# NVlabs/FoundationPose

Hardware: NVIDIA H100
Metric: pose-hypotheses/sec at 640x480 RGB-D, 252 hyp, 5 refine iters (higher is better)
Workload: dtype f16

## Files before the change

foundationpose_b200/csrc/fp_attn_tc.cu:

```cuda
#include "fp_attn.cuh"
#include "fp_common.cuh"
#include "fp_gemm.cuh"
#include "fp_wgmma.cuh"

namespace fp {

int encode_map_f16(CUtensorMap* map, const void* base, int rank, const uint64_t* dims, const uint64_t* strides_bytes,
                   const uint32_t* box);
int num_sms();

namespace {

constexpr int T = 400;
constexpr int DH = 128;
constexpr int kQTiles = (T + 127) / 128;
constexpr int kKeys = 80;
constexpr int kChunks = T / kKeys;
constexpr int kKVSlab = kKeys * 128;
constexpr int kKVStage = 4 * kKVSlab;
constexpr int kKVStages = 3;
constexpr int kQSlab = 128 * 128;
constexpr int kQStage = 2 * kQSlab;
constexpr int kQStages = 2;
constexpr int kOffKV = 0;
constexpr int kOffQ = kOffKV + kKVStages * kKVStage;
constexpr int kOffBar = kOffQ + kQStages * kQStage;
constexpr int kSmem = kOffBar + 256 + 1024;
constexpr int kThreadsTc = 384;

__device__ __forceinline__ void tma_load_3d(const CUtensorMap* map, uint64_t* bar, void* dst, int c0, int c1, int c2) {
  asm volatile(
      "cp.async.bulk.tensor.3d.shared::cluster.global.mbarrier::complete_tx::bytes [%0], [%1, {%3, %4, %5}], [%2];" ::"r"(
          smem_u32(dst)),
      "l"(reinterpret_cast<uint64_t>(map)), "r"(smem_u32(bar)), "r"(c0), "r"(c1), "r"(c2)
      : "memory");
}
__device__ __forceinline__ void tma_store_4d(const CUtensorMap* map, const void* src, int c0, int c1, int c2, int c3) {
  asm volatile("cp.async.bulk.tensor.4d.global.shared::cta.bulk_group [%0, {%2, %3, %4, %5}], [%1];" ::"l"(
                   reinterpret_cast<uint64_t>(map)),
               "r"(smem_u32(src)), "r"(c0), "r"(c1), "r"(c2), "r"(c3)
               : "memory");
}

struct TcParams {
  int q_col, k_col, v_col;
  int group_col_stride;
  float scale_log2e;
  int B, H, G;
};

__global__ void __launch_bounds__(kThreadsTc, 1)
    attn_tc_kernel(const __grid_constant__ CUtensorMap map_kv,
                   const __grid_constant__ CUtensorMap map_q,
                   const __grid_constant__ CUtensorMap map_o,
                   const TcParams p) {
  extern __shared__ uint8_t smem_raw[];
  uint8_t* smem = reinterpret_cast<uint8_t*>((reinterpret_cast<uintptr_t>(smem_raw) + 1023) & ~uintptr_t(1023));
  uint64_t* bars = reinterpret_cast<uint64_t*>(smem + kOffBar);
  uint64_t* q_full = bars;
  uint64_t* q_empty = bars + kQStages;
  uint64_t* kv_full = bars + 2 * kQStages;
  uint64_t* kv_empty = bars + 2 * kQStages + kKVStages;

  const int total = p.B * p.H * p.G * kQTiles;

  if (threadIdx.x == 0) {
    tma_prefetch_desc(&map_kv);
    tma_prefetch_desc(&map_q);
    tma_prefetch_desc(&map_o);
    for (int i = 0; i < kQStages; ++i) {
      mbar_init(&q_full[i], 1);
      mbar_init(&q_empty[i], 2);
    }
    for (int i = 0; i < kKVStages; ++i) {
      mbar_init(&kv_full[i], 1);
      mbar_init(&kv_empty[i], 256);
    }
    mbar_fence_init();
  }
  __syncthreads();
  pdl_trigger();
  pdl_wait();

  auto unit = [&](int u, int& b, int& h, int& g, int& gcol, int& qt) {
    qt = u % kQTiles;
    const int w = u / kQTiles;
    b = w % p.B;
    h = (w / p.B) % p.H;
    g = w / (p.B * p.H);
    gcol = g * p.group_col_stride + h * DH;
  };

  if (threadIdx.x < 128) {
    if (threadIdx.x == 0) {
      int qs = 0, qph = 0, ks = 0, kph = 0;
      for (int u = blockIdx.x; u < total; u += gridDim.x) {
        int b, h, g, gcol, qt;
        unit(u, b, h, g, gcol, qt);
        mbar_wait(&q_empty[qs], qph ^ 1);
        mbar_expect_tx(&q_full[qs], kQStage);
        for (int s = 0; s < 2; ++s)
          tma_load_3d(&map_q, &q_full[qs], smem + kOffQ + qs * kQStage + s * kQSlab, gcol + p.q_col + s * 64, qt * 128, b);
        if (++qs == kQStages) {
          qs = 0;
          qph ^= 1;
        }
        for (int c = 0; c < kChunks; ++c) {
          mbar_wait(&kv_empty[ks], kph ^ 1);
          mbar_expect_tx(&kv_full[ks], kKVStage);
          uint8_t* st = smem + kOffKV + ks * kKVStage;
          for (int s = 0; s < 2; ++s) {
            tma_load_3d(&map_kv, &kv_full[ks], st + s * kKVSlab, gcol + p.k_col + s * 64, c * kKeys, b);
            tma_load_3d(&map_kv, &kv_full[ks], st + (2 + s) * kKVSlab, gcol + p.v_col + s * 64, c * kKeys, b);
          }
          if (++ks == kKVStages) {
            ks = 0;
            kph ^= 1;
          }
        }
      }
    }
    return;
  }

  const int ct = threadIdx.x - 128;
  const int cw = ct >> 7;
  const int lane = threadIdx.x & 31;
  const int r0 = 64 * cw + 16 * ((ct >> 5) & 3) + (lane >> 2);
  const int cq = 2 * (lane & 3);
  const bool leader = ((ct & 127) == 0);
  const float c = p.scale_log2e;
  float s_acc[kKeys / 2], o[DH / 2];
#pragma unroll
  for (int i = 0; i < kKeys / 2; ++i) s_acc[i] = 0.f;
  int qs = 0, qph = 0, ks = 0, kph = 0;
  for (int u = blockIdx.x; u < total; u += gridDim.x) {
    int b, h, g, gcol, qt;
    unit(u, b, h, g, gcol, qt);
#pragma unroll
    for (int i = 0; i < DH / 2; ++i) o[i] = 0.f;
    float m[2] = {-INFINITY, -INFINITY}, l[2] = {0.f, 0.f};
    mbar_wait(&q_full[qs], qph);
    const uint32_t qbase = smem_u32(smem + kOffQ + qs * kQStage) + (uint32_t)cw * 8192u;
    for (int ch = 0; ch < kChunks; ++ch) {
      mbar_wait(&kv_full[ks], kph);
      const uint32_t kvbase = smem_u32(smem + kOffKV + ks * kKVStage);
      wgmma_fence();
#pragma unroll
      for (int kk = 0; kk < 8; ++kk) {
        const int s = kk >> 2, k = kk & 3;
        Wgmma<kKeys>::ss(s_acc, gmma_desc_sw128(qbase + s * kQSlab) + (uint64_t)(2 * k),
                         gmma_desc_sw128(kvbase + s * kKVSlab) + (uint64_t)(2 * k), kk > 0 ? 1u : 0u);
      }
      wgmma_commit();
      wgmma_wait<0>();
      fence_regs(s_acc);
      float mx[2] = {m[0], m[1]};
#pragma unroll
      for (int j = 0; j < kKeys / 8; ++j) {
        mx[0] = fmaxf(mx[0], fmaxf(s_acc[4 * j], s_acc[4 * j + 1]));
        mx[1] = fmaxf(mx[1], fmaxf(s_acc[4 * j + 2], s_acc[4 * j + 3]));
      }
      float mc[2], alpha[2];
#pragma unroll
      for (int hh = 0; hh < 2; ++hh) {
        mx[hh] = fmaxf(mx[hh], __shfl_xor_sync(0xffffffffu, mx[hh], 1));
        mx[hh] = fmaxf(mx[hh], __shfl_xor_sync(0xffffffffu, mx[hh], 2));
        alpha[hh] = exp2f((m[hh] - mx[hh]) * c);
        m[hh] = mx[hh];
        mc[hh] = mx[hh] * c;
        l[hh] *= alpha[hh];
      }
#pragma unroll
      for (int j = 0; j < DH / 8; ++j) {
        o[4 * j] *= alpha[0];
        o[4 * j + 1] *= alpha[0];
        o[4 * j + 2] *= alpha[1];
        o[4 * j + 3] *= alpha[1];
      }
      uint32_t pa[kKeys / 16][4];
#pragma unroll
      for (int j = 0; j < kKeys / 8; ++j) {
#pragma unroll
        for (int hh = 0; hh < 2; ++hh) {
          const float p0 = exp2f(fmaf(s_acc[4 * j + 2 * hh], c, -mc[hh]));
          const float p1 = exp2f(fmaf(s_acc[4 * j + 2 * hh + 1], c, -mc[hh]));
          l[hh] += p0 + p1;
          pa[j >> 1][(j & 1) * 2 + hh] = pack_half2(p0, p1);
        }
      }
      wgmma_fence();
#pragma unroll
      for (int kk = 0; kk < kKeys / 16; ++kk)
        Wgmma<DH>::rs_mn(o, pa[kk], gmma_desc_mn_sw128(kvbase + 2 * kKVSlab + kk * 16 * 128, kKVSlab), 1u);
      wgmma_commit();
      wgmma_wait<0>();
      fence_regs(o);
      mbar_arrive(&kv_empty[ks]);
      if (++ks == kKVStages) {
        ks = 0;
        kph ^= 1;
      }
    }
    float inv[2];
#pragma unroll
    for (int hh = 0; hh < 2; ++hh) {
      l[hh] += __shfl_xor_sync(0xffffffffu, l[hh], 1);
      l[hh] += __shfl_xor_sync(0xffffffffu, l[hh], 2);
      inv[hh] = 1.f / l[hh];
    }
    uint8_t* qst = smem + kOffQ + qs * kQStage;
#pragma unroll
    for (int j = 0; j < DH / 8; ++j) {
#pragma unroll
      for (int hh = 0; hh < 2; ++hh) {
        const int row = r0 + 8 * hh;
        *reinterpret_cast<uint32_t*>(qst + (j >> 3) * kQSlab + row * 128 + ((((uint32_t)j & 7u) ^ (uint32_t)(row & 7)) << 4) +
                                     cq * 2) = pack_half2(o[4 * j + 2 * hh] * inv[hh], o[4 * j + 2 * hh + 1] * inv[hh]);
      }
    }
    asm volatile("fence.proxy.async.shared::cta;" ::: "memory");
    asm volatile("bar.sync %0, 128;" ::"r"(1 + cw) : "memory");
    if (leader) {
      for (int s = 0; s < 2; ++s)
        tma_store_4d(&map_o, qst + s * kQSlab + cw * 8192, h * DH + s * 64, qt * 128 + 64 * cw, b, g);
      asm volatile("cp.async.bulk.commit_group;" ::: "memory");
      asm volatile("cp.async.bulk.wait_group.read 0;" ::: "memory");
      mbar_arrive(&q_empty[qs]);
    }
    if (++qs == kQStages) {
      qs = 0;
      qph ^= 1;
    }
  }
  if (leader) asm volatile("cp.async.bulk.wait_group 0;" ::: "memory");
}

}

int attn_tc_launch(const AttnParams& p, cudaStream_t stream) {
  FP_REQUIRE(p.T == T && p.n_heads == 4, "wgmma attention is specialised for T=400, 4 heads of 128");
  FP_REQUIRE(p.ld_out == 512, "wgmma attention writes [*, 512] rows");
  static std::atomic<unsigned long long> attr_mask{0};
  if (!device_bit_test(attr_mask)) {
    FP_CUDA_OK(cudaFuncSetAttribute(attn_tc_kernel, cudaFuncAttributeMaxDynamicSharedMemorySize, kSmem));
    device_bit_set(attr_mask);
  }
  if (p.B == 0) return 0;
  CUtensorMap mkv, mq, mo;
  const uint64_t E = 2;
  uint64_t d3[3] = {(uint64_t)p.ld, (uint64_t)T, (uint64_t)p.B};
  uint64_t s3[2] = {(uint64_t)p.ld * E, (uint64_t)p.ld * E * T};
  uint32_t bkv[3] = {64, (uint32_t)kKeys, 1}, bq[3] = {64, 128, 1};
  int rc = encode_map_f16(&mkv, p.qkv, 3, d3, s3, bkv);
  if (rc) return rc;
  rc = encode_map_f16(&mq, p.qkv, 3, d3, s3, bq);
  if (rc) return rc;
  uint64_t d4[4] = {512, (uint64_t)T, (uint64_t)p.B, (uint64_t)p.n_groups};
  uint64_t s4[3] = {512 * E, 512 * E * T, (uint64_t)p.out_group_stride * E};
  if (p.n_groups == 1) s4[2] = 512 * E * T * p.B;
  uint32_t bo[4] = {64, 64, 1, 1};
  rc = encode_map_f16(&mo, p.out, 4, d4, s4, bo);
  if (rc) return rc;
  TcParams tp;
  tp.q_col = p.q_off;
  tp.k_col = p.k_off;
  tp.v_col = p.v_off;
  tp.group_col_stride = p.group_col_stride;
  tp.scale_log2e = p.scale * 1.4426950408889634f;
  tp.B = p.B;
  tp.H = p.n_heads;
  tp.G = p.n_groups;
  const int total = p.B * p.n_heads * p.n_groups * kQTiles;
  const int sms = num_sms();
  FP_REQUIRE(sms > 0, "no CUDA device");
  dim3 grid(total < sms ? total : sms);
  FP_CUDA_OK(launch_pdl(attn_tc_kernel, grid, dim3(kThreadsTc), kSmem, stream, 1, mkv, mq, mo, tp));
  note_launches(1);
  FP_CUDA_OK(cudaGetLastError());
  return 0;
}

}
```

foundationpose_b200/csrc/fp_common.cuh:

```cuda
#pragma once
#include <cuda.h>
#include <cuda_fp16.h>
#include <cuda_runtime.h>
#include <stdint.h>
#include <stdio.h>
#include <string.h>

#include <atomic>

namespace fp {

void note_launches(int n);
unsigned long long launch_count();
void set_capturing(bool on);
inline bool device_bit_test(const std::atomic<unsigned long long>& m) {
  int d = 0;
  cudaGetDevice(&d);
  return (m.load(std::memory_order_acquire) >> (d & 63)) & 1ull;
}
inline void device_bit_set(std::atomic<unsigned long long>& m) {
  int d = 0;
  cudaGetDevice(&d);
  m.fetch_or(1ull << (d & 63), std::memory_order_release);
}
int num_sms();

void set_last_error(const char* fmt, ...);
int check_device_ptr(const void* p, const char* what, const char* fn = "fp_pose_errors");
#define FP_CUDA_OK(expr)                                                                   \
  do {                                                                                     \
    cudaError_t _e = (expr);                                                               \
    if (_e != cudaSuccess) {                                                               \
      fp::set_last_error("%s:%d: %s -> %s", __FILE__, __LINE__, #expr, cudaGetErrorString(_e)); \
      return -2;                                                                           \
    }                                                                                      \
  } while (0)
#define FP_REQUIRE(cond, ...)                                                              \
  do {                                                                                     \
    if (!(cond)) {                                                                         \
      fp::set_last_error(__VA_ARGS__);                                                     \
      return -1;                                                                           \
    }                                                                                      \
  } while (0)
#define FP_TRY(expr)     \
  do {                   \
    int _rc = (expr);    \
    if (_rc) return _rc; \
  } while (0)

bool pdl_enabled();
void pdl_skip_next();

template <typename... KArgs, typename... Args>
inline cudaError_t launch_pdl(void (*kernel)(KArgs...), dim3 grid, dim3 block, size_t smem, cudaStream_t stream,
                              int cluster_x, Args... args) {
  cudaLaunchConfig_t cfg;
  memset(&cfg, 0, sizeof(cfg));
  cfg.gridDim = grid;
  cfg.blockDim = block;
  cfg.dynamicSmemBytes = smem;
  cfg.stream = stream;
  cudaLaunchAttribute attr[2];
  int na = 0;
  if (cluster_x > 1) {
    attr[na].id = cudaLaunchAttributeClusterDimension;
    attr[na].val.clusterDim.x = cluster_x;
    attr[na].val.clusterDim.y = 1;
    attr[na].val.clusterDim.z = 1;
    ++na;
  }
  if (pdl_enabled()) {
    attr[na].id = cudaLaunchAttributeProgrammaticStreamSerialization;
    attr[na].val.programmaticStreamSerializationAllowed = 1;
    ++na;
  }
  cfg.attrs = attr;
  cfg.numAttrs = na;
  return cudaLaunchKernelEx(&cfg, kernel, KArgs(args)...);
}

__device__ __forceinline__ void pdl_wait() { asm volatile("griddepcontrol.wait;" ::: "memory"); }
__device__ __forceinline__ void pdl_trigger() { asm volatile("griddepcontrol.launch_dependents;" ::: "memory"); }

__device__ __forceinline__ uint32_t smem_u32(const void* p) {
  return static_cast<uint32_t>(__cvta_generic_to_shared(p));
}

__device__ __forceinline__ void mbar_init(uint64_t* bar, uint32_t count) {
  asm volatile("mbarrier.init.shared::cta.b64 [%0], %1;" ::"r"(smem_u32(bar)), "r"(count));
}
__device__ __forceinline__ void mbar_fence_init() {
  asm volatile("fence.mbarrier_init.release.cluster;" ::: "memory");
}
__device__ __forceinline__ void mbar_expect_tx(uint64_t* bar, uint32_t bytes) {
  asm volatile("mbarrier.arrive.expect_tx.shared::cta.b64 _, [%0], %1;" ::"r"(smem_u32(bar)),
               "r"(bytes)
               : "memory");
}
__device__ __forceinline__ void mbar_arrive(uint64_t* bar) {
  asm volatile("mbarrier.arrive.shared::cta.b64 _, [%0];" ::"r"(smem_u32(bar)) : "memory");
}
__device__ __forceinline__ void mbar_wait(uint64_t* bar, uint32_t parity) {
  asm volatile(
      "{\n\t"
      ".reg .pred P1;\n\t"
      "WAIT_%=:\n\t"
      "mbarrier.try_wait.parity.shared::cta.b64 P1, [%0], %1, %2;\n\t"
      "@P1 bra DONE_%=;\n\t"
      "bra WAIT_%=;\n\t"
      "DONE_%=:\n\t"
      "}" ::"r"(smem_u32(bar)),
      "r"(parity), "r"(0x989680)
      : "memory");
}

__device__ __forceinline__ void tma_load_5d(const CUtensorMap* map, uint64_t* bar, void* dst,
                                            int c0, int c1, int c2, int c3, int c4) {
  asm volatile(
      "cp.async.bulk.tensor.5d.shared::cluster.global.mbarrier::complete_tx::bytes"
      " [%0], [%1, {%3, %4, %5, %6, %7}], [%2];" ::"r"(smem_u32(dst)),
      "l"(reinterpret_cast<uint64_t>(map)), "r"(smem_u32(bar)), "r"(c0), "r"(c1), "r"(c2),
      "r"(c3), "r"(c4)
      : "memory");
}
__device__ __forceinline__ void tma_load_2d(const CUtensorMap* map, uint64_t* bar, void* dst,
                                            int c0, int c1) {
  asm volatile(
      "cp.async.bulk.tensor.2d.shared::cluster.global.mbarrier::complete_tx::bytes"
      " [%0], [%1, {%3, %4}], [%2];" ::"r"(smem_u32(dst)),
      "l"(reinterpret_cast<uint64_t>(map)), "r"(smem_u32(bar)), "r"(c0), "r"(c1)
      : "memory");
}
__device__ __forceinline__ void tma_store_5d(const CUtensorMap* map, const void* src, int c0, int c1, int c2, int c3,
                                             int c4) {
  asm volatile("cp.async.bulk.tensor.5d.global.shared::cta.bulk_group [%0, {%2, %3, %4, %5, %6}], [%1];" ::"l"(
                   reinterpret_cast<uint64_t>(map)),
               "r"(smem_u32(src)), "r"(c0), "r"(c1), "r"(c2), "r"(c3), "r"(c4)
               : "memory");
}
__device__ __forceinline__ void tma_prefetch_desc(const CUtensorMap* map) {
  asm volatile("prefetch.tensormap [%0];" ::"l"(reinterpret_cast<uint64_t>(map)) : "memory");
}

__device__ __forceinline__ uint32_t cluster_nctarank() {
  uint32_t r;
  asm volatile("mov.u32 %0, %%cluster_nctarank;" : "=r"(r));
  return r;
}
__device__ __forceinline__ uint32_t cluster_ctarank() {
  uint32_t r;
  asm volatile("mov.u32 %0, %%cluster_ctarank;" : "=r"(r));
  return r;
}
__device__ __forceinline__ void cluster_sync_all() {
  asm volatile("barrier.cluster.arrive.release.aligned;" ::: "memory");
  asm volatile("barrier.cluster.wait.acquire.aligned;" ::: "memory");
}

template <uint32_t N>
__device__ __forceinline__ void regs_release() {
  asm volatile("setmaxnreg.dec.sync.aligned.u32 %0;" ::"n"(N));
}
template <uint32_t N>
__device__ __forceinline__ void regs_acquire() {
  asm volatile("setmaxnreg.inc.sync.aligned.u32 %0;" ::"n"(N));
}

__device__ __forceinline__ void wgmma_fence() { asm volatile("wgmma.fence.sync.aligned;" ::: "memory"); }
__device__ __forceinline__ void wgmma_commit() { asm volatile("wgmma.commit_group.sync.aligned;" ::: "memory"); }
template <int N>
__device__ __forceinline__ void wgmma_wait() {
  asm volatile("wgmma.wait_group.sync.aligned %0;" ::"n"(N) : "memory");
}
template <int N>
__device__ __forceinline__ void fence_regs(float (&d)[N]) {
#pragma unroll
  for (int i = 0; i < N; ++i) asm volatile("" : "+f"(d[i])::"memory");
}

__device__ __forceinline__ uint64_t gmma_desc_sw128(uint32_t smem_addr, uint32_t sbo = 1024) {
  uint64_t d = 0;
  d |= (uint64_t)((smem_addr & 0x3FFFF) >> 4);
  d |= (uint64_t)1 << 16;
  d |= (uint64_t)(sbo >> 4) << 32;
  d |= (uint64_t)1 << 62;
  return d;
}
__device__ __forceinline__ uint64_t gmma_desc_mn_sw128(uint32_t smem_addr, uint32_t lbo) {
  uint64_t d = 0;
  d |= (uint64_t)((smem_addr & 0x3FFFF) >> 4);
  d |= (uint64_t)((lbo >> 4) & 0x3FFF) << 16;
  d |= (uint64_t)(1024 >> 4) << 32;
  d |= (uint64_t)1 << 62;
  return d;
}
__device__ __forceinline__ uint64_t gmma_desc_linear(uint32_t smem_addr, uint32_t lbo, uint32_t sbo) {
  uint64_t d = 0;
  d |= (uint64_t)((smem_addr & 0x3FFFF) >> 4);
  d |= (uint64_t)(lbo >> 4) << 16;
  d |= (uint64_t)(sbo >> 4) << 32;
  return d;
}

__device__ __forceinline__ void ldsm_x4_trans(uint32_t addr, uint32_t (&r)[4]) {
  asm volatile("ldmatrix.sync.aligned.m8n8.x4.trans.shared.b16 {%0, %1, %2, %3}, [%4];"
               : "=r"(r[0]), "=r"(r[1]), "=r"(r[2]), "=r"(r[3])
               : "r"(addr)
               : "memory");
}
__device__ __forceinline__ void stsm_x4_trans(uint32_t addr, const uint32_t (&r)[4]) {
  asm volatile("stmatrix.sync.aligned.m8n8.x4.trans.shared.b16 [%0], {%1, %2, %3, %4};" ::"r"(addr), "r"(r[0]),
               "r"(r[1]), "r"(r[2]), "r"(r[3])
               : "memory");
}

__device__ __forceinline__ uint32_t pack_half2(float a, float b) {
  __half2 h = __floats2half2_rn(a, b);
  return *reinterpret_cast<uint32_t*>(&h);
}

}
```

foundationpose_b200/csrc/fp_linear.cu:

```cuda
#include <stdlib.h>
#include <string.h>

#include "fp_common.cuh"
#include "fp_gemm.cuh"
#include "fp_wgmma.cuh"

namespace fp {

int encode_map_f16(CUtensorMap* map, const void* base, int rank, const uint64_t* dims, const uint64_t* strides_bytes,
                   const uint32_t* box);

constexpr int kLwsK = 512;
constexpr int kLwsKBlocks = kLwsK / 64;
constexpr int kLwsRows = 64;
constexpr int kLwsCols = 128;
constexpr int kLwsThreads = 384;
constexpr int kLwsBoxBytes = kLwsCols * 64 * 2;
constexpr int kLwsPanelBytes = kLwsKBlocks * kLwsBoxBytes;
constexpr int kLwsStages = kLwsKBlocks;
constexpr int kLwsStageBytes = kLwsRows * 64 * 2;
constexpr int kLwsSlabBytes = kLwsRows * 64 * 2;
constexpr int kLwsSlabs = 4;
constexpr int kLwsSmemBytes =
    kLwsPanelBytes + kLwsStages * kLwsStageBytes + kLwsSlabs * kLwsSlabBytes + 1024  + 256 ;
static_assert(kLwsSmemBytes <= 232448, "the weight-stationary linear kernel exceeds the 227 KB opt-in shared memory");
static_assert((2 * kLwsStages + 4) * 8 <= 256, "the mbarriers must fit their 256 bytes");

constexpr uint32_t kOrderBar = 2;
constexpr uint32_t kWgBar = 4;

struct LinearWsParams {
  int row_tiles;
  int total;
  const float* bias;
  int has_res;
  int relu;
};

__device__ __forceinline__ void named_sync(uint32_t id, uint32_t count) {
  asm volatile("bar.sync %0, %1;" ::"r"(id), "r"(count) : "memory");
}
__device__ __forceinline__ void named_arrive(uint32_t id, uint32_t count) {
  asm volatile("bar.arrive %0, %1;" ::"r"(id), "r"(count) : "memory");
}

__global__ void __launch_bounds__(kLwsThreads, 1)
    linear_ws_kernel(const __grid_constant__ CUtensorMap map_a, const __grid_constant__ CUtensorMap map_w,
                     const __grid_constant__ CUtensorMap map_out, const __grid_constant__ CUtensorMap map_res,
                     const __grid_constant__ LinearWsParams p) {
  extern __shared__ uint8_t smem_raw[];
  uint8_t* smem = smem_raw + ((1024u - (smem_u32(smem_raw) & 1023u)) & 1023u);
  uint8_t* panel = smem;
  uint8_t* ring = panel + kLwsPanelBytes;
  uint8_t* staging = ring + kLwsStages * kLwsStageBytes;
  uint64_t* bars = reinterpret_cast<uint64_t*>(staging + kLwsSlabs * kLwsSlabBytes);
  uint64_t* full = bars;
  uint64_t* empty = bars + kLwsStages;
  uint64_t* panel_full = bars + 2 * kLwsStages;
  uint64_t* panel_empty = panel_full + 1;
  uint64_t* res_full = panel_full + 2;

  const int i0 = (int)((long long)blockIdx.x * p.total / gridDim.x);
  const int n = (int)((long long)(blockIdx.x + 1) * p.total / gridDim.x) - i0;
  const int panel0 = i0 / p.row_tiles;
  const int jb = min(n, (panel0 + 1) * p.row_tiles - i0);
  const bool reload = jb < n;

  if (threadIdx.x == 0) {
    tma_prefetch_desc(&map_a);
    tma_prefetch_desc(&map_w);
    tma_prefetch_desc(&map_out);
    if (p.has_res) tma_prefetch_desc(&map_res);
    for (int s = 0; s < kLwsStages; ++s) {
      mbar_init(&full[s], 1);
      mbar_init(&empty[s], 128);
    }
    mbar_init(panel_full, 1);
    mbar_init(panel_empty, 256);
    mbar_init(&res_full[0], 1);
    mbar_init(&res_full[1], 1);
    mbar_fence_init();
    mbar_expect_tx(panel_full, kLwsPanelBytes);
    for (int kb = 0; kb < kLwsKBlocks; ++kb)
      tma_load_2d(&map_w, panel_full, panel + kb * kLwsBoxBytes, kb * 64, panel0 * kLwsCols);
  }
  __syncthreads();
  pdl_trigger();
  pdl_wait();

  if (threadIdx.x < 128) {
    if (threadIdx.x == 0) {
      for (int j = 0; j < n; ++j) {
        if (j == jb) {
          mbar_wait(panel_empty, 0);
          mbar_expect_tx(panel_full, kLwsPanelBytes);
          for (int kb = 0; kb < kLwsKBlocks; ++kb)
            tma_load_2d(&map_w, panel_full, panel + kb * kLwsBoxBytes, kb * 64, (panel0 + 1) * kLwsCols);
        }
        const int row0 = ((i0 + j) % p.row_tiles) * kLwsRows;
        for (int kb = 0; kb < kLwsKBlocks; ++kb) {
          mbar_wait(&empty[kb], (uint32_t)((j & 1) ^ 1));
          mbar_expect_tx(&full[kb], kLwsStageBytes);
          tma_load_2d(&map_a, &full[kb], ring + kb * kLwsStageBytes, kb * 64, row0);
        }
      }
    }
    return;
  }

  const int ct = threadIdx.x - 128;
  const int w = ct >> 7;
  const int lane = threadIdx.x & 31;
  const int r0 = 16 * ((ct >> 5) & 3) + (lane >> 2);
  const int cq = 2 * (lane & 3);
  const bool leader = (ct & 127) == 0;
  uint8_t* slabs = staging + w * 2 * kLwsSlabBytes;
  if (reload && w >= jb) mbar_arrive(panel_empty);
  float acc[64];
#pragma unroll
  for (int i = 0; i < 64; ++i) acc[i] = 0.f;
  for (int j = w, it = 0; j < n; j += 2, ++it) {
    const int item = i0 + j;
    const int pn = item / p.row_tiles;
    const int row0 = (item - pn * p.row_tiles) * kLwsRows;
    if (j > 0) named_sync(kOrderBar + w, 256);
    mbar_wait(panel_full, j >= jb ? 1u : 0u);
    for (int kb = 0; kb < kLwsKBlocks; ++kb) {
      mbar_wait(&full[kb], (uint32_t)(j & 1));
      const uint64_t da = gmma_desc_sw128(smem_u32(ring + kb * kLwsStageBytes));
      const uint64_t db = gmma_desc_sw128(smem_u32(panel + kb * kLwsBoxBytes));
      wgmma_fence();
#pragma unroll
      for (int k = 0; k < 4; ++k)
        Wgmma<128>::ss(acc, da + (uint64_t)(2 * k), db + (uint64_t)(2 * k), (kb > 0 || k > 0) ? 1u : 0u);
      wgmma_commit();
      if (kb == 0 && leader) {
        asm volatile("cp.async.bulk.wait_group.read 0;" ::: "memory");
        if (p.has_res) {
          mbar_expect_tx(&res_full[w], 2 * kLwsSlabBytes);
          for (int s = 0; s < 2; ++s)
            tma_load_5d(&map_res, &res_full[w], slabs + s * kLwsSlabBytes, pn * kLwsCols + 64 * s, row0, 0, 0, 0);
        }
      }
      if (kb > 0) {
        wgmma_wait<1>();
        mbar_arrive(&empty[kb - 1]);
      }
    }
    if (j + 1 < n) named_arrive(kOrderBar + (w ^ 1), 256);
    wgmma_wait<0>();
    fence_regs(acc);
    mbar_arrive(&empty[kLwsKBlocks - 1]);
    if (reload && j < jb && j + 2 >= jb) mbar_arrive(panel_empty);

    const float* bias = p.bias + pn * kLwsCols;
    if (p.has_res) mbar_wait(&res_full[w], (uint32_t)(it & 1));
    else named_sync(kWgBar + w, 128);
#pragma unroll
    for (int b = 0; b < 2; ++b) {
      uint8_t* slab = slabs + b * kLwsSlabBytes;
#pragma unroll
      for (int jh = 0; jh < 8; jh += 4) {
        float2 bb[4];
        __half2 rv[4][2];
#pragma unroll
        for (int jl = 0; jl < 4; ++jl) {
          bb[jl] = __ldg(reinterpret_cast<const float2*>(bias + 64 * b + 8 * (jh + jl) + cq));
          if (p.has_res) {
#pragma unroll
            for (int h = 0; h < 2; ++h) {
              const int row = r0 + 8 * h;
              rv[jl][h] = *reinterpret_cast<const __half2*>(slab + row * 128 + (((uint32_t)(jh + jl) ^ (uint32_t)(row & 7)) << 4) + cq * 2);
            }
          }
        }
#pragma unroll
        for (int jl = 0; jl < 4; ++jl) {
          const int jc = 8 * b + jh + jl;
#pragma unroll
          for (int h = 0; h < 2; ++h) {
            const int row = r0 + 8 * h;
            uint32_t* cell = reinterpret_cast<uint32_t*>(slab + row * 128 + (((uint32_t)(jh + jl) ^ (uint32_t)(row & 7)) << 4) + cq * 2);
            float a0 = acc[4 * jc + 2 * h] + bb[jl].x, a1 = acc[4 * jc + 2 * h + 1] + bb[jl].y;
            if (p.has_res) {
              const float2 r = __half22float2(rv[jl][h]);
              a0 += r.x;
              a1 += r.y;
            }
            if (p.relu) {
              a0 = fmaxf(a0, 0.f);
              a1 = fmaxf(a1, 0.f);
            }
            *cell = pack_half2(a0, a1);
          }
        }
      }
    }
    asm volatile("fence.proxy.async.shared::cta;" ::: "memory");
    named_sync(kWgBar + w, 128);
    if (leader) {
      for (int s = 0; s < 2; ++s)
        tma_store_5d(&map_out, slabs + s * kLwsSlabBytes, pn * kLwsCols + 64 * s, row0, 0, 0, 0);
      asm volatile("cp.async.bulk.commit_group;" ::: "memory");
    }
  }
  if (leader) asm volatile("cp.async.bulk.wait_group 0;" ::: "memory");
}

static bool linear_ws_enabled() {
  const char* e = getenv("FPOSE_LINEAR_WS");
  return !(e && e[0] == '0');
}

constexpr int kLinearWsMinItemsPerCta = 8;

bool linear_ws_takes(const GemmLayer& L) {
  if (L.kind != LK_LINEAR || L.Cin != kLwsK || L.Cout % kLwsCols != 0 || L.out_split != 0 || L.post_add ||
      !linear_ws_enabled())
    return false;
  const int sms = num_sms();
  const int panels = L.Cout / kLwsCols;
  const long long items = (long long)panels * ((L.Win + kLwsRows - 1) / kLwsRows);
  return sms > 0 && panels <= sms && items >= (long long)kLinearWsMinItemsPerCta * sms;
}

int linear_ws_launch(const GemmLayer& L, cudaStream_t stream) {
  const uint64_t E = 2;
  const int M = L.Win;
  LinearWsParams p;
  memset(&p, 0, sizeof(p));
  p.row_tiles = (M + kLwsRows - 1) / kLwsRows;
  p.total = (L.Cout / kLwsCols) * p.row_tiles;
  p.bias = L.bias;
  p.has_res = L.res != nullptr;
  p.relu = L.relu;
  CUtensorMap ma, mw, mo, mr;
  {
    const uint64_t d[2] = {(uint64_t)kLwsK, (uint64_t)M}, s[1] = {(uint64_t)kLwsK * E};
    const uint32_t b[2] = {64, kLwsRows};
    if (int rc = encode_map_f16(&ma, L.in, 2, d, s, b)) return rc;
  }
  {
    const uint64_t d[2] = {(uint64_t)kLwsK, (uint64_t)L.Cout}, s[1] = {(uint64_t)kLwsK * E};
    const uint32_t b[2] = {64, kLwsCols};
    if (int rc = encode_map_f16(&mw, L.w, 2, d, s, b)) return rc;
  }
  auto rows_map = [&](CUtensorMap* m, const void* base, int ld) {
    const uint64_t row = (uint64_t)ld * E;
    const uint64_t d[5] = {(uint64_t)ld, (uint64_t)M, 1, 1, 1}, s[4] = {row, row * M, row * M, row * M};
    const uint32_t b[5] = {64, kLwsRows, 1, 1, 1};
    return encode_map_f16(m, base, 5, d, s, b);
  };
  if (int rc = rows_map(&mo, L.out, L.out_ld)) return rc;
  mr = mo;
  if (L.res) {
    if (int rc = rows_map(&mr, L.res, L.res_ld)) return rc;
  }

  static std::atomic<unsigned long long> attr_mask{0};
  if (!device_bit_test(attr_mask)) {
    FP_CUDA_OK(cudaFuncSetAttribute(linear_ws_kernel, cudaFuncAttributeMaxDynamicSharedMemorySize, kLwsSmemBytes));
    device_bit_set(attr_mask);
  }
  const int sms = num_sms();
  FP_REQUIRE(sms > 0, "no CUDA device");
  const int grid = p.total < sms ? p.total : sms;
  prof_mark_begin(0, 2.0 * (double)M * L.Cout * kLwsK, stream);
  FP_CUDA_OK(launch_pdl(linear_ws_kernel, dim3(grid), dim3(kLwsThreads), kLwsSmemBytes, stream, 1, ma, mw, mo, mr, p));
  prof_mark_end(stream);
  note_launches(1);
  FP_CUDA_OK(cudaGetLastError());
  return 0;
}

}
```

Baseline: 3836.

## Pipeline QK and PV wgmma in attention with split K/V barriers

Splits the K/V ring into separate K and V stages with their own barriers. The consumer loop now issues the next chunk's QK^T wgmma alongside the current PV wgmma, overlapping softmax with tensor-core work in FA3 style. It also adds producer/consumer register reallocation, a dedicated output staging buffer so the Q stage is released early, and rotates the pass index per CTA with a grid rounded to a multiple of kPasses. In the last Q pass the second consumer warpgroup skips padded rows, which lowers wasted compute on the 400-token tail but leaves that warpgroup idle and adds synchronization complexity.

```diff
diff --git a/foundationpose_b200/csrc/fp_attn_tc.cu b/foundationpose_b200/csrc/fp_attn_tc.cu
--- a/foundationpose_b200/csrc/fp_attn_tc.cu
+++ b/foundationpose_b200/csrc/fp_attn_tc.cu
@@ -13,20 +13,28 @@
 
 constexpr int T = 400;
 constexpr int DH = 128;
-constexpr int kQTiles = (T + 127) / 128;
+constexpr int kPasses = (T + 127) / 128;
 constexpr int kKeys = 80;
 constexpr int kChunks = T / kKeys;
 constexpr int kKVSlab = kKeys * 128;
-constexpr int kKVStage = 4 * kKVSlab;
+constexpr int kKVStage = 2 * kKVSlab;
 constexpr int kKVStages = 3;
 constexpr int kQSlab = 128 * 128;
 constexpr int kQStage = 2 * kQSlab;
 constexpr int kQStages = 2;
-constexpr int kOffKV = 0;
-constexpr int kOffQ = kOffKV + kKVStages * kKVStage;
-constexpr int kOffBar = kOffQ + kQStages * kQStage;
+constexpr int kOSlab = 64 * 128;
+constexpr int kOStage = 2 * kOSlab;
+constexpr int kOffK = 0;
+constexpr int kOffV = kOffK + kKVStages * kKVStage;
+constexpr int kOffQ = kOffV + kKVStages * kKVStage;
+constexpr int kOffO = kOffQ + kQStages * kQStage;
+constexpr int kOffBar = kOffO + 2 * kOStage;
 constexpr int kSmem = kOffBar + 256 + 1024;
+static_assert(kSmem <= 232448, "the attention kernel exceeds the 227 KB opt-in shared memory");
 constexpr int kThreadsTc = 384;
+constexpr int kProducerRegs = 40;
+constexpr int kConsumerRegs = 232;
+constexpr uint32_t kWgBar = 1;
 
 __device__ __forceinline__ void tma_load_3d(const CUtensorMap* map, uint64_t* bar, void* dst, int c0, int c1, int c2) {
   asm volatile(
@@ -48,6 +56,64 @@
   float scale_log2e;
   int B, H, G;
 };
+
+__device__ __forceinline__ void issue_s(float (&s_acc)[kKeys / 2], uint32_t qbase, uint32_t kbase) {
+#pragma unroll
+  for (int kk = 0; kk < 8; ++kk) {
+    const int s = kk >> 2, k = kk & 3;
+    Wgmma<kKeys>::ss(s_acc, gmma_desc_sw128(qbase + s * kQSlab) + (uint64_t)(2 * k),
+                     gmma_desc_sw128(kbase + s * kKVSlab) + (uint64_t)(2 * k), kk > 0 ? 1u : 0u);
+  }
+}
+__device__ __forceinline__ void issue_pv(float (&o)[DH / 2], const uint32_t (&pa)[kKeys / 16][4], uint32_t vbase) {
+#pragma unroll
+  for (int kk = 0; kk < kKeys / 16; ++kk)
+    Wgmma<DH>::rs_mn(o, pa[kk], gmma_desc_mn_sw128(vbase + kk * 16 * 128, kKVSlab), 1u);
+}
+__device__ __forceinline__ void softmax_step(float (&s_acc)[kKeys / 2], float (&m)[2], float (&l)[2], float (&alpha)[2],
+                                             float c) {
+  float mx[2] = {m[0], m[1]};
+#pragma unroll
+  for (int j = 0; j < kKeys / 8; ++j) {
+    mx[0] = fmaxf(mx[0], fmaxf(s_acc[4 * j], s_acc[4 * j + 1]));
+    mx[1] = fmaxf(mx[1], fmaxf(s_acc[4 * j + 2], s_acc[4 * j + 3]));
+  }
+  float mc[2];
+#pragma unroll
+  for (int hh = 0; hh < 2; ++hh) {
+    mx[hh] = fmaxf(mx[hh], __shfl_xor_sync(0xffffffffu, mx[hh], 1));
+    mx[hh] = fmaxf(mx[hh], __shfl_xor_sync(0xffffffffu, mx[hh], 2));
+    alpha[hh] = exp2f((m[hh] - mx[hh]) * c);
+    m[hh] = mx[hh];
+    mc[hh] = mx[hh] * c;
+    l[hh] *= alpha[hh];
+  }
+#pragma unroll
+  for (int j = 0; j < kKeys / 8; ++j) {
+#pragma unroll
+    for (int hh = 0; hh < 2; ++hh) {
+      const float p0 = exp2f(fmaf(s_acc[4 * j + 2 * hh], c, -mc[hh]));
+      const float p1 = exp2f(fmaf(s_acc[4 * j + 2 * hh + 1], c, -mc[hh]));
+      l[hh] += p0 + p1;
+      s_acc[4 * j + 2 * hh] = p0;
+      s_acc[4 * j + 2 * hh + 1] = p1;
+    }
+  }
+}
+__device__ __forceinline__ void rescale_and_pack(float (&o)[DH / 2], const float (&alpha)[2],
+                                                 const float (&s_acc)[kKeys / 2], uint32_t (&pa)[kKeys / 16][4]) {
+#pragma unroll
+  for (int j = 0; j < DH / 8; ++j) {
+    o[4 * j] *= alpha[0];
+    o[4 * j + 1] *= alpha[0];
+    o[4 * j + 2] *= alpha[1];
+    o[4 * j + 3] *= alpha[1];
+  }
+#pragma unroll
+  for (int j = 0; j < kKeys / 8; ++j)
+#pragma unroll
+    for (int hh = 0; hh < 2; ++hh) pa[j >> 1][(j & 1) * 2 + hh] = pack_half2(s_acc[4 * j + 2 * hh], s_acc[4 * j + 2 * hh + 1]);
+}
 
 __global__ void __launch_bounds__(kThreadsTc, 1)
     attn_tc_kernel(const __grid_constant__ CUtensorMap map_kv,
@@ -59,10 +125,12 @@
   uint64_t* bars = reinterpret_cast<uint64_t*>(smem + kOffBar);
   uint64_t* q_full = bars;
   uint64_t* q_empty = bars + kQStages;
-  uint64_t* kv_full = bars + 2 * kQStages;
-  uint64_t* kv_empty = bars + 2 * kQStages + kKVStages;
-
-  const int total = p.B * p.H * p.G * kQTiles;
+  uint64_t* k_full = bars + 2 * kQStages;
+  uint64_t* k_empty = k_full + kKVStages;
+  uint64_t* v_full = k_full + 2 * kKVStages;
+  uint64_t* v_empty = k_full + 3 * kKVStages;
+
+  const int total = p.B * p.H * p.G * kPasses;
 
   if (threadIdx.x == 0) {
     tma_prefetch_desc(&map_kv);
@@ -70,11 +138,13 @@
     tma_prefetch_desc(&map_o);
     for (int i = 0; i < kQStages; ++i) {
       mbar_init(&q_full[i], 1);
-      mbar_init(&q_empty[i], 2);
+      mbar_init(&q_empty[i], 256);
     }
     for (int i = 0; i < kKVStages; ++i) {
-      mbar_init(&kv_full[i], 1);
-      mbar_init(&kv_empty[i], 256);
+      mbar_init(&k_full[i], 1);
+      mbar_init(&k_empty[i], 256);
+      mbar_init(&v_full[i], 1);
+      mbar_init(&v_empty[i], 256);
     }
     mbar_fence_init();
   }
@@ -82,9 +152,9 @@
   pdl_trigger();
   pdl_wait();
 
-  auto unit = [&](int u, int& b, int& h, int& g, int& gcol, int& qt) {
-    qt = u % kQTiles;
-    const int w = u / kQTiles;
+  auto unit = [&](int u, int& b, int& h, int& g, int& gcol, int& pass) {
+    pass = (u + u / (int)gridDim.x) % kPasses;
+    const int w = u / kPasses;
     b = w % p.B;
     h = (w / p.B) % p.H;
     g = w / (p.B * p.H);
@@ -92,27 +162,31 @@
   };
 
   if (threadIdx.x < 128) {
+    regs_release<kProducerRegs>();
     if (threadIdx.x == 0) {
       int qs = 0, qph = 0, ks = 0, kph = 0;
       for (int u = blockIdx.x; u < total; u += gridDim.x) {
-        int b, h, g, gcol, qt;
-        unit(u, b, h, g, gcol, qt);
+        int b, h, g, gcol, pass;
+        unit(u, b, h, g, gcol, pass);
         mbar_wait(&q_empty[qs], qph ^ 1);
         mbar_expect_tx(&q_full[qs], kQStage);
         for (int s = 0; s < 2; ++s)
-          tma_load_3d(&map_q, &q_full[qs], smem + kOffQ + qs * kQStage + s * kQSlab, gcol + p.q_col + s * 64, qt * 128, b);
+          tma_load_3d(&map_q, &q_full[qs], smem + kOffQ + qs * kQStage + s * kQSlab, gcol + p.q_col + s * 64, pass * 128, b);
         if (++qs == kQStages) {
           qs = 0;
           qph ^= 1;
         }
         for (int c = 0; c < kChunks; ++c) {
-          mbar_wait(&kv_empty[ks], kph ^ 1);
-          mbar_expect_tx(&kv_full[ks], kKVStage);
-          uint8_t* st = smem + kOffKV + ks * kKVStage;
-          for (int s = 0; s < 2; ++s) {
-            tma_load_3d(&map_kv, &kv_full[ks], st + s * kKVSlab, gcol + p.k_col + s * 64, c * kKeys, b);
-            tma_load_3d(&map_kv, &kv_full[ks], st + (2 + s) * kKVSlab, gcol + p.v_col + s * 64, c * kKeys, b);
-          }
+          mbar_wait(&k_empty[ks], kph ^ 1);
+          mbar_expect_tx(&k_full[ks], kKVStage);
+          for (int s = 0; s < 2; ++s)
+            tma_load_3d(&map_kv, &k_full[ks], smem + kOffK + ks * kKVStage + s * kKVSlab, gcol + p.k_col + s * 64,
+                        c * kKeys, b);
+          mbar_wait(&v_empty[ks], kph ^ 1);
+          mbar_expect_tx(&v_full[ks], kKVStage);
+          for (int s = 0; s < 2; ++s)
+            tma_load_3d(&map_kv, &v_full[ks], smem + kOffV + ks * kKVStage + s * kKVSlab, gcol + p.v_col + s * 64,
+                        c * kKeys, b);
           if (++ks == kKVStages) {
             ks = 0;
             kph ^= 1;
@@ -123,110 +197,106 @@
     return;
   }
 
+  regs_acquire<kConsumerRegs>();
   const int ct = threadIdx.x - 128;
   const int cw = ct >> 7;
   const int lane = threadIdx.x & 31;
-  const int r0 = 64 * cw + 16 * ((ct >> 5) & 3) + (lane >> 2);
+  const int r0 = 16 * ((ct >> 5) & 3) + (lane >> 2);
   const int cq = 2 * (lane & 3);
   const bool leader = ((ct & 127) == 0);
   const float c = p.scale_log2e;
+  uint8_t* ost = smem + kOffO + cw * kOStage;
   float s_acc[kKeys / 2], o[DH / 2];
-#pragma unroll
-  for (int i = 0; i < kKeys / 2; ++i) s_acc[i] = 0.f;
+  uint32_t pa[kKeys / 16][4];
   int qs = 0, qph = 0, ks = 0, kph = 0;
+  auto next_kv = [&]() {
+    if (++ks == kKVStages) {
+      ks = 0;
+      kph ^= 1;
+    }
+  };
   for (int u = blockIdx.x; u < total; u += gridDim.x) {
-    int b, h, g, gcol, qt;
-    unit(u, b, h, g, gcol, qt);
-#pragma unroll
-    for (int i = 0; i < DH / 2; ++i) o[i] = 0.f;
-    float m[2] = {-INFINITY, -INFINITY}, l[2] = {0.f, 0.f};
-    mbar_wait(&q_full[qs], qph);
-    const uint32_t qbase = smem_u32(smem + kOffQ + qs * kQStage) + (uint32_t)cw * 8192u;
-    for (int ch = 0; ch < kChunks; ++ch) {
-      mbar_wait(&kv_full[ks], kph);
-      const uint32_t kvbase = smem_u32(smem + kOffKV + ks * kKVStage);
+    int b, h, g, gcol, pass;
+    unit(u, b, h, g, gcol, pass);
+    if (pass == kPasses - 1 && cw == 1) {
+      mbar_wait(&q_full[qs], qph);
+      mbar_arrive(&q_empty[qs]);
+      for (int ch = 0; ch < kChunks; ++ch) {
+        mbar_wait(&k_full[ks], kph);
+        mbar_arrive(&k_empty[ks]);
+        mbar_wait(&v_full[ks], kph);
+        mbar_arrive(&v_empty[ks]);
+        next_kv();
+      }
+    } else {
+#pragma unroll
+      for (int i = 0; i < DH / 2; ++i) o[i] = 0.f;
+      float m[2] = {-INFINITY, -INFINITY}, l[2] = {0.f, 0.f}, alpha[2];
+      mbar_wait(&q_full[qs], qph);
+      const uint32_t qbase = smem_u32(smem + kOffQ + qs * kQStage) + (uint32_t)cw * 8192u;
+      mbar_wait(&k_full[ks], kph);
+      int vs = ks, vph = kph;
+      next_kv();
       wgmma_fence();
-#pragma unroll
-      for (int kk = 0; kk < 8; ++kk) {
-        const int s = kk >> 2, k = kk & 3;
-        Wgmma<kKeys>::ss(s_acc, gmma_desc_sw128(qbase + s * kQSlab) + (uint64_t)(2 * k),
-                         gmma_desc_sw128(kvbase + s * kKVSlab) + (uint64_t)(2 * k), kk > 0 ? 1u : 0u);
-      }
+      issue_s(s_acc, qbase, smem_u32(smem + kOffK + vs * kKVStage));
       wgmma_commit();
       wgmma_wait<0>();
       fence_regs(s_acc);
-      float mx[2] = {m[0], m[1]};
-#pragma unroll
-      for (int j = 0; j < kKeys / 8; ++j) {
-        mx[0] = fmaxf(mx[0], fmaxf(s_acc[4 * j], s_acc[4 * j + 1]));
-        mx[1] = fmaxf(mx[1], fmaxf(s_acc[4 * j + 2], s_acc[4 * j + 3]));
-      }
-      float mc[2], alpha[2];
-#pragma unroll
-      for (int hh = 0; hh < 2; ++hh) {
-        mx[hh] = fmaxf(mx[hh], __shfl_xor_sync(0xffffffffu, mx[hh], 1));
-        mx[hh] = fmaxf(mx[hh], __shfl_xor_sync(0xffffffffu, mx[hh], 2));
-        alpha[hh] = exp2f((m[hh] - mx[hh]) * c);
-        m[hh] = mx[hh];
-        mc[hh] = mx[hh] * c;
-        l[hh] *= alpha[hh];
-      }
-#pragma unroll
-      for (int j = 0; j < DH / 8; ++j) {
-        o[4 * j] *= alpha[0];
-        o[4 * j + 1] *= alpha[0];
-        o[4 * j + 2] *= alpha[1];
-        o[4 * j + 3] *= alpha[1];
-      }
-      uint32_t pa[kKeys / 16][4];
-#pragma unroll
-      for (int j = 0; j < kKeys / 8; ++j) {
-#pragma unroll
-        for (int hh = 0; hh < 2; ++hh) {
-          const float p0 = exp2f(fmaf(s_acc[4 * j + 2 * hh], c, -mc[hh]));
-          const float p1 = exp2f(fmaf(s_acc[4 * j + 2 * hh + 1], c, -mc[hh]));
-          l[hh] += p0 + p1;
-          pa[j >> 1][(j & 1) * 2 + hh] = pack_half2(p0, p1);
-        }
-      }
+      mbar_arrive(&k_empty[vs]);
+      softmax_step(s_acc, m, l, alpha, c);
+      rescale_and_pack(o, alpha, s_acc, pa);
+      for (int ch = 1; ch < kChunks; ++ch) {
+        mbar_wait(&k_full[ks], kph);
+        mbar_wait(&v_full[vs], vph);
+        wgmma_fence();
+        issue_s(s_acc, qbase, smem_u32(smem + kOffK + ks * kKVStage));
+        wgmma_commit();
+        issue_pv(o, pa, smem_u32(smem + kOffV + vs * kKVStage));
+        wgmma_commit();
+        wgmma_wait<1>();
+        fence_regs(s_acc);
+        mbar_arrive(&k_empty[ks]);
+        if (ch == kChunks - 1) mbar_arrive(&q_empty[qs]);
+        softmax_step(s_acc, m, l, alpha, c);
+        wgmma_wait<0>();
+        fence_regs(o);
+        mbar_arrive(&v_empty[vs]);
+        rescale_and_pack(o, alpha, s_acc, pa);
+        vs = ks;
+        vph = kph;
+        next_kv();
+      }
+      mbar_wait(&v_full[vs], vph);
       wgmma_fence();
-#pragma unroll
-      for (int kk = 0; kk < kKeys / 16; ++kk)
-        Wgmma<DH>::rs_mn(o, pa[kk], gmma_desc_mn_sw128(kvbase + 2 * kKVSlab + kk * 16 * 128, kKVSlab), 1u);
+      issue_pv(o, pa, smem_u32(smem + kOffV + vs * kKVStage));
       wgmma_commit();
       wgmma_wait<0>();
       fence_regs(o);
-      mbar_arrive(&kv_empty[ks]);
-      if (++ks == kKVStages) {
-        ks = 0;
-        kph ^= 1;
-      }
-    }
-    float inv[2];
-#pragma unroll
-    for (int hh = 0; hh < 2; ++hh) {
-      l[hh] += __shfl_xor_sync(0xffffffffu, l[hh], 1);
-      l[hh] += __shfl_xor_sync(0xffffffffu, l[hh], 2);
-      inv[hh] = 1.f / l[hh];
-    }
-    uint8_t* qst = smem + kOffQ + qs * kQStage;
-#pragma unroll
-    for (int j = 0; j < DH / 8; ++j) {
+      mbar_arrive(&v_empty[vs]);
+      float inv[2];
 #pragma unroll
       for (int hh = 0; hh < 2; ++hh) {
-        const int row = r0 + 8 * hh;
-        *reinterpret_cast<uint32_t*>(qst + (j >> 3) * kQSlab + row * 128 + ((((uint32_t)j & 7u) ^ (uint32_t)(row & 7)) << 4) +
-                                     cq * 2) = pack_half2(o[4 * j + 2 * hh] * inv[hh], o[4 * j + 2 * hh + 1] * inv[hh]);
-      }
-    }
-    asm volatile("fence.proxy.async.shared::cta;" ::: "memory");
-    asm volatile("bar.sync %0, 128;" ::"r"(1 + cw) : "memory");
-    if (leader) {
-      for (int s = 0; s < 2; ++s)
-        tma_store_4d(&map_o, qst + s * kQSlab + cw * 8192, h * DH + s * 64, qt * 128 + 64 * cw, b, g);
-      asm volatile("cp.async.bulk.commit_group;" ::: "memory");
-      asm volatile("cp.async.bulk.wait_group.read 0;" ::: "memory");
-      mbar_arrive(&q_empty[qs]);
+        l[hh] += __shfl_xor_sync(0xffffffffu, l[hh], 1);
+        l[hh] += __shfl_xor_sync(0xffffffffu, l[hh], 2);
+        inv[hh] = 1.f / l[hh];
+      }
+      if (leader) asm volatile("cp.async.bulk.wait_group.read 0;" ::: "memory");
+      named_sync(kWgBar + cw, 128);
+#pragma unroll
+      for (int j = 0; j < DH / 8; ++j) {
+#pragma unroll
+        for (int hh = 0; hh < 2; ++hh) {
+          const int row = r0 + 8 * hh;
+          *reinterpret_cast<uint32_t*>(ost + (j >> 3) * kOSlab + row * 128 + ((((uint32_t)j & 7u) ^ (uint32_t)(row & 7)) << 4) +
+                                       cq * 2) = pack_half2(o[4 * j + 2 * hh] * inv[hh], o[4 * j + 2 * hh + 1] * inv[hh]);
+        }
+      }
+      asm volatile("fence.proxy.async.shared::cta;" ::: "memory");
+      named_sync(kWgBar + cw, 128);
+      if (leader) {
+        for (int s = 0; s < 2; ++s) tma_store_4d(&map_o, ost + s * kOSlab, h * DH + s * 64, pass * 128 + 64 * cw, b, g);
+        asm volatile("cp.async.bulk.commit_group;" ::: "memory");
+      }
     }
     if (++qs == kQStages) {
       qs = 0;
@@ -271,10 +341,11 @@
   tp.B = p.B;
   tp.H = p.n_heads;
   tp.G = p.n_groups;
-  const int total = p.B * p.n_heads * p.n_groups * kQTiles;
+  const int total = p.B * p.n_heads * p.n_groups * kPasses;
   const int sms = num_sms();
   FP_REQUIRE(sms > 0, "no CUDA device");
-  dim3 grid(total < sms ? total : sms);
+  const int cap = sms >= kPasses ? sms / kPasses * kPasses : kPasses;
+  dim3 grid(total < cap ? total : cap);
   FP_CUDA_OK(launch_pdl(attn_tc_kernel, grid, dim3(kThreadsTc), kSmem, stream, 1, mkv, mq, mo, tp));
   note_launches(1);
   FP_CUDA_OK(cudaGetLastError());
diff --git a/foundationpose_b200/csrc/fp_common.cuh b/foundationpose_b200/csrc/fp_common.cuh
--- a/foundationpose_b200/csrc/fp_common.cuh
+++ b/foundationpose_b200/csrc/fp_common.cuh
@@ -166,6 +166,13 @@
   asm volatile("setmaxnreg.inc.sync.aligned.u32 %0;" ::"n"(N));
 }
 
+__device__ __forceinline__ void named_sync(uint32_t id, uint32_t count) {
+  asm volatile("bar.sync %0, %1;" ::"r"(id), "r"(count) : "memory");
+}
+__device__ __forceinline__ void named_arrive(uint32_t id, uint32_t count) {
+  asm volatile("bar.arrive %0, %1;" ::"r"(id), "r"(count) : "memory");
+}
+
 __device__ __forceinline__ void wgmma_fence() { asm volatile("wgmma.fence.sync.aligned;" ::: "memory"); }
 __device__ __forceinline__ void wgmma_commit() { asm volatile("wgmma.commit_group.sync.aligned;" ::: "memory"); }
 template <int N>
diff --git a/foundationpose_b200/csrc/fp_linear.cu b/foundationpose_b200/csrc/fp_linear.cu
--- a/foundationpose_b200/csrc/fp_linear.cu
+++ b/foundationpose_b200/csrc/fp_linear.cu
@@ -37,13 +37,6 @@
   int relu;
 };
 
-__device__ __forceinline__ void named_sync(uint32_t id, uint32_t count) {
-  asm volatile("bar.sync %0, %1;" ::"r"(id), "r"(count) : "memory");
-}
-__device__ __forceinline__ void named_arrive(uint32_t id, uint32_t count) {
-  asm volatile("bar.arrive %0, %1;" ::"r"(id), "r"(count) : "memory");
-}
-
 __global__ void __launch_bounds__(kLwsThreads, 1)
     linear_ws_kernel(const __grid_constant__ CUtensorMap map_a, const __grid_constant__ CUtensorMap map_w,
                      const __grid_constant__ CUtensorMap map_out, const __grid_constant__ CUtensorMap map_res,
```

Result: no change. 3848, median of 6 (+0.3%).
